# yangcaoai/CoDA_NeurIPS2023

Measured on NVIDIA H100. Metric: training scenes/sec (20k-pt SUN-RGBD synth, 256 queries), higher is better.
Workload: dtype fp32

## Files before the change

### coda_neurips2023_b200/csrc/sa_mlp_kernels.cu

```cuda
#include <cuda_bf16.h>
#include <math.h>
#include <stdint.h>

#include "../../include/coda_sa_mlp.h"
#include "coda_common.cuh"
#include "operand_split.cuh"

namespace {

constexpr int THREADS = 256;
constexpr int MAX_BLOCKS = 132 * 4;

__host__ __device__ inline bool channels_ok(int c) { return c >= 4 && c <= 1024 && c % 4 == 0 && THREADS % (c / 4) == 0; }

__host__ inline unsigned grid_for(long long rows, int c) {
  const long long per_iter = THREADS / (c / 4);
  const long long need = (rows + per_iter - 1) / per_iter;
  return (unsigned)(need < MAX_BLOCKS ? (need > 0 ? need : 1) : MAX_BLOCKS);
}

struct Affine4 {
  float4 mean, invstd, gamma, beta;
};
__device__ __forceinline__ Affine4 load_affine(const float *mean, const float *invstd, const float *gamma,
// ... 146 lines not shown
  warp_partials_sum(nblocks, c, ch, partial, s, q);
  if ((threadIdx.x & 31) != 0) return;
  sums[ch] = s;
  sums[c + ch] = q;
}
__global__ void __launch_bounds__(256)
bn_finalize_sums_kernel(long long rows, int c, int cpad, const double *__restrict__ sums, float eps, float momentum,
                        float *running_mean, float *running_var, const float *__restrict__ gamma,
                        const float *__restrict__ beta, float *__restrict__ mean, float *__restrict__ invstd,
                        float *__restrict__ scale, float *__restrict__ shift) {
  const int ch = blockIdx.x * blockDim.x + threadIdx.x;
  if (ch >= cpad) return;
  if (ch >= c) {
    if (scale) { scale[ch] = 0.f; shift[ch] = 0.f; }
    return;
  }
  const double n = (double)rows, m = sums[ch] / n;
  double var = sums[c + ch] / n - m * m;
  if (var < 0.0) var = 0.0;
  const float is = (float)(1.0 / sqrt(var + (double)eps));
  mean[ch] = (float)m;
  invstd[ch] = is;
  if (running_mean) running_mean[ch] = (1.0f - momentum) * running_mean[ch] + momentum * (float)m;
  if (running_var) running_var[ch] = (1.0f - momentum) * running_var[ch] + momentum * (float)(var * (n / fmax(n - 1.0, 1.0)));
  if (scale) {
    const float sc = gamma[ch] * is;
    scale[ch] = sc;
    shift[ch] = beta[ch] - (float)m * sc;
  }
}

__global__ void bn_bwd_coefs_kernel(int c, int cpad, long long rows, const float *__restrict__ mean,
                                    const float *__restrict__ invstd, const float *__restrict__ gamma,
                                    const float *__restrict__ s1, const float *__restrict__ s2,
                                    float *__restrict__ alpha, float *__restrict__ beta) {
  const int ch = blockIdx.x * blockDim.x + threadIdx.x;
  if (ch >= cpad) return;
  if (ch >= c) { alpha[ch] = 0.f; beta[ch] = 0.f; return; }
  const float inv_n = 1.0f / (float)rows;
  const float sc = gamma[ch] * invstd[ch];
  const float a = -sc * invstd[ch] * (s2[ch] * inv_n);
  alpha[ch] = a;
  beta[ch] = -sc * (s1[ch] * inv_n) - a * mean[ch];
}

__global__ void __launch_bounds__(THREADS)
colsum_partial_kernel(long long rows, int c, const float *__restrict__ x, float *__restrict__ partial) {
  __shared__ float4 red[THREADS];
  const int cq = c >> 2, c4 = threadIdx.x % cq, slot = threadIdx.x / cq, nslots = THREADS / cq;
  float4 acc[1] = {make_float4(0.f, 0.f, 0.f, 0.f)};
  for (long long r = (long long)blockIdx.x * nslots + slot; r < rows; r += (long long)gridDim.x * nslots) {
    const float4 v = __ldg(reinterpret_cast<const float4 *>(x + r * c) + c4);
    acc[0].x += v.x; acc[0].y += v.y; acc[0].z += v.z; acc[0].w += v.w;
  }
  reduce_slots<1>(acc, cq, slot, c4, red);
  if (slot == 0) reinterpret_cast<float4 *>(partial + (size_t)blockIdx.x * c)[c4] = acc[0];
}
__global__ void __launch_bounds__(256)
colsum_finalize_kernel(int nblocks, int c, const float *__restrict__ partial, float *__restrict__ out) {
  const int ch = blockIdx.x * 8 + (threadIdx.x >> 5), lane = threadIdx.x & 31;
  if (ch >= c) return;
  float a = 0.f;
  for (int k = lane; k < nblocks; k += 32) a += partial[(size_t)k * c + ch];
#pragma unroll
  for (int o = 16; o > 0; o >>= 1) a += __shfl_xor_sync(0xffffffffu, a, o);
  if (lane == 0) out[ch] = a;
}

template <int NS>
__global__ void __launch_bounds__(THREADS)
bn_relu_pack_kernel(long long rows, int c, const float *__restrict__ y, const float *__restrict__ mean,
                    const float *__restrict__ invstd, const float *__restrict__ gamma, const float *__restrict__ beta,
                    __nv_bfloat16 *__restrict__ planes) {
  const int cq = c >> 2, c4 = threadIdx.x % cq, slot = threadIdx.x / cq, nslots = THREADS / cq;
  const Affine4 a = load_affine(mean, invstd, gamma, beta, c4);
  const size_t plane_stride = (size_t)rows * c;
  for (long long r = (long long)blockIdx.x * nslots + slot; r < rows; r += (long long)gridDim.x * nslots) {
    const float4 z = bn4(xhat4(__ldg(reinterpret_cast<const float4 *>(y + r * c) + c4), a), a);
    coda::split_store4<NS>(make_float4(fmaxf(z.x, 0.f), fmaxf(z.y, 0.f), fmaxf(z.z, 0.f), fmaxf(z.w, 0.f)),
                           planes + r * c + c4 * 4, plane_stride);
  }
}

__global__ void __launch_bounds__(THREADS)
bn_relu_maxpool_kernel(long long groups, int group, int c, const float *__restrict__ y, const float *__restrict__ mean,
                       const float *__restrict__ invstd, const float *__restrict__ gamma,
                       const float *__restrict__ beta, float *__restrict__ pooled, unsigned char *__restrict__ argmax) {
  __shared__ float4 sval[THREADS];
  __shared__ uchar4 sidx[THREADS];
  const int cq = c >> 2, c4 = threadIdx.x % cq, slot = threadIdx.x / cq, nslots = THREADS / cq;
  const Affine4 a = load_affine(mean, invstd, gamma, beta, c4);
  for (long long g = blockIdx.x; g < groups; g += gridDim.x) {
    float4 best = make_float4(-INFINITY, -INFINITY, -INFINITY, -INFINITY);
    uchar4 bi = make_uchar4(0, 0, 0, 0);
    for (int i = slot; i < group; i += nslots) {
      const float4 zz = bn4(xhat4(__ldg(reinterpret_cast<const float4 *>(y + (g * group + i) * c) + c4), a), a);
      const float4 z = make_float4(fmaxf(zz.x, 0.f), fmaxf(zz.y, 0.f), fmaxf(zz.z, 0.f), fmaxf(zz.w, 0.f));
      if (z.x > best.x) { best.x = z.x; bi.x = (unsigned char)i; }
      if (z.y > best.y) { best.y = z.y; bi.y = (unsigned char)i; }
      if (z.z > best.z) { best.z = z.z; bi.z = (unsigned char)i; }
      if (z.w > best.w) { best.w = z.w; bi.w = (unsigned char)i; }
    }
    __syncthreads();
    sval[threadIdx.x] = best;
    sidx[threadIdx.x] = bi;
    __syncthreads();
    if (slot == 0) {
      for (int s = 1; s < nslots; ++s) {
        const float4 o = sval[s * cq + c4];
        const uchar4 oi = sidx[s * cq + c4];
        if (o.x > best.x || (o.x == best.x && oi.x < bi.x)) { best.x = o.x; bi.x = oi.x; }
        if (o.y > best.y || (o.y == best.y && oi.y < bi.y)) { best.y = o.y; bi.y = oi.y; }
        if (o.z > best.z || (o.z == best.z && oi.z < bi.z)) { best.z = o.z; bi.z = oi.z; }
        if (o.w > best.w || (o.w == best.w && oi.w < bi.w)) { best.w = o.w; bi.w = oi.w; }
      }
      reinterpret_cast<float4 *>(pooled + g * c)[c4] = best;
      reinterpret_cast<uchar4 *>(argmax + g * c)[c4] = bi;
    }
  }
}

__global__ void __launch_bounds__(THREADS)
bn_relu_bwd_reduce_kernel(long long rows, int c, const float *__restrict__ y, const float *__restrict__ dz,
                          const float *__restrict__ mean, const float *__restrict__ invstd,
                          const float *__restrict__ gamma, const float *__restrict__ beta, float *__restrict__ partial) {
  __shared__ float4 red[THREADS];
  const int cq = c >> 2, c4 = threadIdx.x % cq, slot = threadIdx.x / cq, nslots = THREADS / cq;
  const Affine4 a = load_affine(mean, invstd, gamma, beta, c4);
  float4 acc[2] = {make_float4(0.f, 0.f, 0.f, 0.f), make_float4(0.f, 0.f, 0.f, 0.f)};
  for (long long r = (long long)blockIdx.x * nslots + slot; r < rows; r += (long long)gridDim.x * nslots) {
    const float4 xh = xhat4(__ldg(reinterpret_cast<const float4 *>(y + r * c) + c4), a);
    const float4 z = bn4(xh, a);
    float4 d = __ldg(reinterpret_cast<const float4 *>(dz + r * c) + c4);
    d.x = z.x > 0.f ? d.x : 0.f; d.y = z.y > 0.f ? d.y : 0.f; d.z = z.z > 0.f ? d.z : 0.f; d.w = z.w > 0.f ? d.w : 0.f;
    acc[0].x += d.x; acc[0].y += d.y; acc[0].z += d.z; acc[0].w += d.w;
    acc[1].x = fmaf(d.x, xh.x, acc[1].x); acc[1].y = fmaf(d.y, xh.y, acc[1].y);
    acc[1].z = fmaf(d.z, xh.z, acc[1].z); acc[1].w = fmaf(d.w, xh.w, acc[1].w);
  }
  reduce_slots<2>(acc, cq, slot, c4, red);
  if (slot == 0) {
    float4 *p = reinterpret_cast<float4 *>(partial + (size_t)blockIdx.x * 2 * c);
    p[c4] = acc[0];
    p[cq + c4] = acc[1];
  }
}
__global__ void __launch_bounds__(THREADS)
bn_relu_bwd_reduce_pooled_kernel(long long groups, int group, int c, const float *__restrict__ y,
                                 const float *__restrict__ dpooled, const unsigned char *__restrict__ argmax,
                                 const float *__restrict__ mean, const float *__restrict__ invstd,
                                 const float *__restrict__ gamma, const float *__restrict__ beta,
                                 float *__restrict__ partial, float *__restrict__ dprime) {
  __shared__ float4 red[THREADS];
  const int cq = c >> 2, c4 = threadIdx.x % cq, slot = threadIdx.x / cq, nslots = THREADS / cq;
  const Affine4 a = load_affine(mean, invstd, gamma, beta, c4);
  float4 acc[2] = {make_float4(0.f, 0.f, 0.f, 0.f), make_float4(0.f, 0.f, 0.f, 0.f)};
  for (long long g = (long long)blockIdx.x * nslots + slot; g < groups; g += (long long)gridDim.x * nslots) {
    const uchar4 id = __ldg(reinterpret_cast<const uchar4 *>(argmax + g * c) + c4);
    const float *base = y + g * group * c + c4 * 4;
    const float4 v = make_float4(__ldg(base + (size_t)id.x * c), __ldg(base + (size_t)id.y * c + 1),
                                 __ldg(base + (size_t)id.z * c + 2), __ldg(base + (size_t)id.w * c + 3));
    const float4 xh = xhat4(v, a);
    const float4 z = bn4(xh, a);
    float4 d = __ldg(reinterpret_cast<const float4 *>(dpooled + g * c) + c4);
    d.x = z.x > 0.f ? d.x : 0.f; d.y = z.y > 0.f ? d.y : 0.f; d.z = z.z > 0.f ? d.z : 0.f; d.w = z.w > 0.f ? d.w : 0.f;
    if (dprime)
      reinterpret_cast<float4 *>(dprime + g * c)[c4] =
          make_float4(a.gamma.x * a.invstd.x * d.x, a.gamma.y * a.invstd.y * d.y, a.gamma.z * a.invstd.z * d.z,
                      a.gamma.w * a.invstd.w * d.w);
    acc[0].x += d.x; acc[0].y += d.y; acc[0].z += d.z; acc[0].w += d.w;
    acc[1].x = fmaf(d.x, xh.x, acc[1].x); acc[1].y = fmaf(d.y, xh.y, acc[1].y);
    acc[1].z = fmaf(d.z, xh.z, acc[1].z); acc[1].w = fmaf(d.w, xh.w, acc[1].w);
  }
  reduce_slots<2>(acc, cq, slot, c4, red);
  if (slot == 0) {
    float4 *p = reinterpret_cast<float4 *>(partial + (size_t)blockIdx.x * 2 * c);
    p[c4] = acc[0];
    p[cq + c4] = acc[1];
  }
}
__global__ void __launch_bounds__(256)
sums_finalize_kernel(int nblocks, int c, const float *__restrict__ partial, float *__restrict__ s1,
                     float *__restrict__ s2) {
  const int ch = blockIdx.x * 8 + (threadIdx.x >> 5);
  if (ch >= c) return;
  double a, b;
  warp_partials_sum(nblocks, c, ch, partial, a, b);
  if ((threadIdx.x & 31) == 0) {
    s1[ch] = (float)a;
    s2[ch] = (float)b;
  }
}

struct BwdCoef4 {
  float4 k, m1, m2;
};
__device__ __forceinline__ BwdCoef4 load_coef(const Affine4 &a, const float *s1, const float *s2, int c4, float inv_n) {
  const float4 t1 = __ldg(reinterpret_cast<const float4 *>(s1) + c4), t2 = __ldg(reinterpret_cast<const float4 *>(s2) + c4);
  BwdCoef4 q;
  q.k = make_float4(a.gamma.x * a.invstd.x, a.gamma.y * a.invstd.y, a.gamma.z * a.invstd.z, a.gamma.w * a.invstd.w);
  q.m1 = make_float4(t1.x * inv_n, t1.y * inv_n, t1.z * inv_n, t1.w * inv_n);
  q.m2 = make_float4(t2.x * inv_n, t2.y * inv_n, t2.z * inv_n, t2.w * inv_n);
// ... 123 lines not shown
  bn_stats_finalize_affine_kernel<<<(cpad + 7) / 8, 256, 0, s>>>((int)grid, rows, c, cpad, scratch, eps, momentum,
                                                                    running_mean, running_var, gamma, beta, mean,
                                                                    invstd, scale, shift);
  return coda::launch_status();
}

int coda_bn_stats_finalize(int nblocks, long long rows, int c, const float *partial, float eps, float momentum,
                           float *running_mean, float *running_var, const float *gamma, const float *beta,
                           float *mean, float *invstd, float *scale, float *shift, void *stream) {
  if (nblocks <= 0 || rows <= 0 || c <= 0 || !partial || !mean || !invstd) return CODA_EINVAL;
  if ((scale != nullptr) != (shift != nullptr) || (scale && (!gamma || !beta))) return CODA_EINVAL;
  const int cpad = (c + 63) / 64 * 64;
  bn_stats_finalize_affine_kernel<<<(cpad + 7) / 8, 256, 0, (cudaStream_t)stream>>>(
      nblocks, rows, c, cpad, partial, eps, momentum, running_mean, running_var, gamma, beta, mean, invstd, scale, shift);
  return coda::launch_status();
}

int coda_bn_rows_sums(long long rows, int c, const float *y, double *sums, float *scratch, void *stream) {
  if (rows <= 0 || !channels_ok(c) || !y || !sums || !scratch) return CODA_EINVAL;
  cudaStream_t s = (cudaStream_t)stream;
  const unsigned grid = grid_for(rows, c);
  bn_stats_partial_kernel<<<grid, THREADS, 0, s>>>(rows, c, y, scratch);
  bn_sums_f64_kernel<<<(c + 7) / 8, 256, 0, s>>>((int)grid, c, scratch, sums);
  return coda::launch_status();
}

int coda_bn_partials_sums(int nblocks, int c, const float *partial, double *sums, void *stream) {
  if (nblocks <= 0 || c <= 0 || !partial || !sums) return CODA_EINVAL;
  bn_sums_f64_kernel<<<(c + 7) / 8, 256, 0, (cudaStream_t)stream>>>(nblocks, c, partial, sums);
  return coda::launch_status();
}

int coda_bn_stats_finalize_sums(long long rows, int c, const double *sums, float eps, float momentum,
                                float *running_mean, float *running_var, const float *gamma, const float *beta,
                                float *mean, float *invstd, float *scale, float *shift, void *stream) {
  if (rows <= 0 || c <= 0 || !sums || !mean || !invstd) return CODA_EINVAL;
  if ((scale != nullptr) != (shift != nullptr) || (scale && (!gamma || !beta))) return CODA_EINVAL;
  const int cpad = scale ? (c + 63) / 64 * 64 : c;
  bn_finalize_sums_kernel<<<(cpad + 127) / 128, 128, 0, (cudaStream_t)stream>>>(
      rows, c, cpad, sums, eps, momentum, running_mean, running_var, gamma, beta, mean, invstd, scale, shift);
  return coda::launch_status();
}

int coda_bn_bwd_coefs(int c, long long rows, const float *mean, const float *invstd, const float *gamma,
                      const float *s1, const float *s2, float *alpha, float *beta, void *stream) {
  if (c <= 0 || rows <= 0 || !mean || !invstd || !gamma || !s1 || !s2 || !alpha || !beta) return CODA_EINVAL;
  const int cpad = (c + 63) / 64 * 64;
  bn_bwd_coefs_kernel<<<(cpad + 127) / 128, 128, 0, (cudaStream_t)stream>>>(c, cpad, rows, mean, invstd, gamma, s1, s2,
                                                                           alpha, beta);
  return coda::launch_status();
}

int coda_rows_colsum(long long rows, int c, const float *x, float *out, float *scratch, void *stream) {
  if (rows <= 0 || !channels_ok(c) || !x || !out || !scratch) return CODA_EINVAL;
  cudaStream_t s = (cudaStream_t)stream;
  unsigned grid = grid_for(rows, c);
  if (grid > 132) grid = 132;
  colsum_partial_kernel<<<grid, THREADS, 0, s>>>(rows, c, x, scratch);
  colsum_finalize_kernel<<<(c + 7) / 8, 256, 0, s>>>((int)grid, c, scratch, out);
  return coda::launch_status();
}

int coda_bn_relu_pack_rows(long long rows, int c, int nsplit, const float *y, const float *mean,
                           const float *invstd, const float *gamma, const float *beta, void *planes,
                           void *stream) {
  if (rows < 0 || !channels_ok(c) || c % 64 != 0 || nsplit < 1 || nsplit > 3) return CODA_EINVAL;
  if (rows == 0) return CODA_OK;
  if (!y || !mean || !invstd || !gamma || !beta || !planes) return CODA_EINVAL;
  cudaStream_t s = (cudaStream_t)stream;
  const unsigned grid = grid_for(rows, c);
  __nv_bfloat16 *p = (__nv_bfloat16 *)planes;
  if (nsplit == 1) bn_relu_pack_kernel<1><<<grid, THREADS, 0, s>>>(rows, c, y, mean, invstd, gamma, beta, p);
  else if (nsplit == 2) bn_relu_pack_kernel<2><<<grid, THREADS, 0, s>>>(rows, c, y, mean, invstd, gamma, beta, p);
  else bn_relu_pack_kernel<3><<<grid, THREADS, 0, s>>>(rows, c, y, mean, invstd, gamma, beta, p);
  return coda::launch_status();
}

int coda_bn_relu_maxpool_rows(long long groups, int group, int c, const float *y, const float *mean,
                              const float *invstd, const float *gamma, const float *beta, float *pooled,
                              unsigned char *argmax, void *stream) {
  if (groups < 0 || group < 1 || group > 256 || !channels_ok(c)) return CODA_EINVAL;
  if (groups == 0) return CODA_OK;
  if (!y || !mean || !invstd || !gamma || !beta || !pooled || !argmax) return CODA_EINVAL;
  const unsigned grid = (unsigned)(groups < 132 * 8 ? groups : 132 * 8);
  bn_relu_maxpool_kernel<<<grid, THREADS, 0, (cudaStream_t)stream>>>(groups, group, c, y, mean, invstd, gamma, beta,
                                                                    pooled, argmax);
  return coda::launch_status();
}

int coda_bn_relu_bwd_reduce(long long rows, int c, const float *y, const float *dz, const float *mean,
                            const float *invstd, const float *gamma, const float *beta, float *s1, float *s2,
                            float *scratch, void *stream) {
  if (rows <= 0 || !channels_ok(c) || !y || !dz || !mean || !invstd || !gamma || !beta || !s1 || !s2 || !scratch)
    return CODA_EINVAL;
  cudaStream_t s = (cudaStream_t)stream;
  const unsigned grid = grid_for(rows, c);
  bn_relu_bwd_reduce_kernel<<<grid, THREADS, 0, s>>>(rows, c, y, dz, mean, invstd, gamma, beta, scratch);
  sums_finalize_kernel<<<(c + 7) / 8, 256, 0, s>>>((int)grid, c, scratch, s1, s2);
  return coda::launch_status();
}

int coda_bn_relu_bwd_reduce_pooled(long long groups, int group, int c, const float *y, const float *dpooled,
                                   const unsigned char *argmax, const float *mean, const float *invstd,
                                   const float *gamma, const float *beta, float *s1, float *s2, float *scratch,
                                   float *dprime, void *stream) {
  if (groups <= 0 || group < 1 || group > 256 || !channels_ok(c) || !y || !dpooled || !argmax || !mean || !invstd ||
      !gamma || !beta || !s1 || !s2 || !scratch)
    return CODA_EINVAL;
  cudaStream_t s = (cudaStream_t)stream;
  const unsigned grid = grid_for(groups, c);
  bn_relu_bwd_reduce_pooled_kernel<<<grid, THREADS, 0, s>>>(groups, group, c, y, dpooled, argmax, mean, invstd, gamma,
                                                           beta, scratch, dprime);
  sums_finalize_kernel<<<(c + 7) / 8, 256, 0, s>>>((int)grid, c, scratch, s1, s2);
  return coda::launch_status();
}

int coda_bn_relu_bwd_pack(long long rows, int c, int nsplit, const float *y, const float *dz,
                          const float *dpooled, const unsigned char *argmax, int group, const float *mean,
                          const float *invstd, const float *gamma, const float *beta, const float *s1,
                          const float *s2, void *planes, void *stream) {
  if (rows < 0 || !channels_ok(c) || c % 64 != 0 || nsplit < 1 || nsplit > 3) return CODA_EINVAL;
  if (rows == 0) return CODA_OK;
  if (!y || !mean || !invstd || !gamma || !beta || !s1 || !s2 || !planes) return CODA_EINVAL;
  const bool pooled = dz == nullptr;
  if (pooled && (!dpooled || !argmax || group < 1 || group > 256 || rows % group != 0)) return CODA_EINVAL;
  cudaStream_t s = (cudaStream_t)stream;
  const unsigned grid = grid_for(rows, c);
  __nv_bfloat16 *p = (__nv_bfloat16 *)planes;
#define CODA_LAUNCH(NS, P) \
  bn_relu_bwd_pack_kernel<NS, P><<<grid, THREADS, 0, s>>>(rows, c, y, dz, dpooled, argmax, group, mean, invstd, gamma, \
                                                          beta, s1, s2, p)
  if (pooled) {
    if (nsplit == 1) CODA_LAUNCH(1, true); else if (nsplit == 2) CODA_LAUNCH(2, true); else CODA_LAUNCH(3, true);
  } else {
    if (nsplit == 1) CODA_LAUNCH(1, false); else if (nsplit == 2) CODA_LAUNCH(2, false); else CODA_LAUNCH(3, false);
  }
#undef CODA_LAUNCH
  return coda::launch_status();
}

int coda_bn_relu_bwd_small_k(long long rows, int cin, int cout, const float *y, const float *dz, const float *mean,
                             const float *invstd, const float *gamma, const float *beta, const float *s1,
                             const float *s2, const float *x, float *dw, float *scratch, void *stream) {
  if (rows <= 0 || cin < 1 || cin > 8 || !channels_ok(cout)) return CODA_EINVAL;
  if (!y || !dz || !mean || !invstd || !gamma || !beta || !s1 || !s2 || !x || !dw || !scratch) return CODA_EINVAL;
  cudaStream_t s = (cudaStream_t)stream;
  const unsigned grid = grid_for(rows, cout);
#define CODA_CASE(K)                                                                                              \
  case K:                                                                                                         \
    bn_relu_bwd_small_k_kernel<K><<<grid, THREADS, 0, s>>>(rows, cout, y, dz, mean, invstd, gamma, beta, s1, s2, x, \
                                                           scratch);                                             \
    break;
  switch (cin) { CODA_CASE(1) CODA_CASE(2) CODA_CASE(3) CODA_CASE(4) CODA_CASE(5) CODA_CASE(6) CODA_CASE(7) CODA_CASE(8) }
#undef CODA_CASE
  dw_finalize_kernel<<<(cin * cout + 127) / 128, 128, 0, s>>>((int)grid, cin * cout, scratch, dw);
  return coda::launch_status();
}

}
```

### coda_neurips2023_b200/csrc/gemm_sm90.cu

```cuda
#include "../../include/coda_gemm.h"
#include "sm90_primitives.cuh"

using namespace coda;

namespace {

template <int NSPLIT>
__global__ void __launch_bounds__(256)
pack_rows_kernel(long long rows, int k, int kpad, long long src_row_stride, const float *__restrict__ src,
                 float scale, __nv_bfloat16 *__restrict__ planes, long long plane_stride) {
  const long long idx = (long long)blockIdx.x * blockDim.x + threadIdx.x;
  if (idx >= rows * kpad) return;
  const long long r = idx / kpad;
  const int c = (int)(idx - r * kpad);
  const float x = c < k ? __ldg(src + r * src_row_stride + c) * scale : 0.f;
  split_store<NSPLIT>(x, planes + idx, (size_t)plane_stride);
}

template <int NSPLIT>
__global__ void __launch_bounds__(256)
pack_rows_vec4_kernel(long long rows, int k, int kpad, long long src_row_stride, const float *__restrict__ src,
                      float scale, __nv_bfloat16 *__restrict__ planes, long long plane_stride) {
  const int kq = kpad >> 2;
  const long long idx = (long long)blockIdx.x * blockDim.x + threadIdx.x;
// ... 253 lines not shown
      for (int kb = 0; kb < nkb; ++kb, ++it) {
        const int s = it % STAGES;
        mbar_wait(&empty_bar[s], ((it / STAGES) & 1u) ^ 1u);
        if (elect_one_sync()) {
          mbar_arrive_expect_tx(&full_bar[s], (uint32_t)STAGE);
          unsigned char *st = smem + (size_t)s * STAGE;
          tma_load_3d(st, &maps.a[0], &full_bar[s], kb * BK, m0, 0);
          tma_load_3d(st + A_TILE, &maps.b[0], &full_bar[s], kb * BK, n0, 0);
        }
        __syncwarp();
      }
    }
    return;
  }
  setmaxnreg_inc<PP_MMA_REGS>();

  const int wg = warp >> 2, wl = warp & 3;
  const int g = lane >> 2, t = lane & 3;
  float acc[2][BN / 2];
  uint32_t it = (uint32_t)(wg * nkb);
  for (int w = blockIdx.x + wg * gridDim.x; w < ntiles; w += 2 * gridDim.x, it += 2 * nkb) {
    int m0, n0;
    decode(w, m0, n0);
    const bool other_next = w + (int)gridDim.x < ntiles;
    if (wg == 1 || w != (int)blockIdx.x) bar_sync(1 + wg, 256);
    for (int kb = 0; kb < nkb; ++kb) {
      const uint32_t i = it + kb;
      const int s = i % STAGES;
      mbar_wait(&full_bar[s], (i / STAGES) & 1u);
      unsigned char *st = smem + (size_t)s * STAGE;
      acc_fence(acc[0]);
      acc_fence(acc[1]);
      wgmma_fence();
      const uint64_t ad = gmma_desc_k_sw128(st), bd = gmma_desc_k_sw128(st + A_TILE);
#pragma unroll
      for (int kk = 0; kk < BK / 16; ++kk) {
        const uint64_t b = gmma_desc_advance(bd, kk * 32);
        Wgmma<BN, true>::template ss<0, 0>(acc[0], gmma_desc_advance(ad, kk * 32), b, (kb | kk) != 0);
        Wgmma<BN, true>::template ss<0, 0>(acc[1], gmma_desc_advance(ad, 8192 + kk * 32), b, (kb | kk) != 0);
      }
      wgmma_commit();
      if (kb == nkb - 1 && other_next) bar_arrive(1 + (wg ^ 1), 256);
      wgmma_wait<1>();
      acc_fence(acc[0]);
      acc_fence(acc[1]);
      if (kb > 0 && (threadIdx.x & 127) == 0) mbar_arrive(&empty_bar[(i - 1) % STAGES]);
    }

    float2 bv[BN / 8];
    if (EPI != PP_NONE) {
#pragma unroll
      for (int cc = 0; cc < BN / 8; ++cc) bv[cc] = __ldg(reinterpret_cast<const float2 *>(bias + n0 + cc * 8 + 2 * t));
    }
    wgmma_wait<0>();
    acc_fence(acc[0]);
    acc_fence(acc[1]);
    if ((threadIdx.x & 127) == 0) mbar_arrive(&empty_bar[(it + nkb - 1) % STAGES]);

#pragma unroll
    for (int h = 0; h < 2; ++h) {
#pragma unroll
      for (int r = 0; r < 2; ++r) {
        const int row = m0 + h * 64 + wl * 16 + g + 8 * r;
        if (row >= m) continue;
        __half *crow = c + (size_t)row * ldc + n0 + 2 * t;
        const __half *rrow = EPI == PP_BIAS_RES ? residual + (size_t)row * ldr + n0 + 2 * t : nullptr;
#pragma unroll
        for (int cc = 0; cc < BN / 8; ++cc) {
          float v0 = acc[h][cc * 4 + r * 2], v1 = acc[h][cc * 4 + r * 2 + 1];
          if (EPI != PP_NONE) { v0 += bv[cc].x; v1 += bv[cc].y; }
          if (EPI == PP_BIAS_GELU) { v0 = apply_act(v0, 2); v1 = apply_act(v1, 2); }
          if (EPI == PP_BIAS_RES) {
            const __half2 rv = *reinterpret_cast<const __half2 *>(rrow + cc * 8);
            v0 += __low2float(rv);
            v1 += __high2float(rv);
          }
          *reinterpret_cast<__half2 *>(crow + cc * 8) = __floats2half2_rn(v0, v1);
        }
      }
    }
  }
}

template <int NSPLIT, int BN, int STAGES, bool FP16, bool MN = false>
int launch_gemm(const GemmMaps &maps, int batch, int m, int n, int kpad, int b_batched, const float *bias, int relu,
                void *c_out, long long ldc, long long c_batch_stride, cudaStream_t s, int out_half = 0,
                const void *residual = nullptr, long long ldr = 0) {
  float *c = reinterpret_cast<float *>(c_out);
  const int sms = sm_count();
  const long long tiles = (long long)((m + BM - 1) / BM) * ((n + BN - 1) / BN) * batch;
  const int nkb_total = kpad / BK;
  int ksplit = 1;
  if (!relu && !out_half && tiles < sms && nkb_total >= 32) {
    ksplit = (int)((2 * sms + tiles - 1) / tiles);
    if (ksplit > nkb_total / 8) ksplit = nkb_total / 8;
    if (ksplit < 1) ksplit = 1;
    const int per = (nkb_total + ksplit - 1) / ksplit;
    ksplit = (nkb_total + per - 1) / per;
  }
  if (residual && (!FP16 || !out_half || batch != 1 || (ldr & 7) != 0 || ((uintptr_t)residual & 15) != 0))
    return CODA_EINVAL;
  float *partial = nullptr;
  if (ksplit > 1) {
    const int st = split_scratch((size_t)tiles * ksplit * BM * BN, s, &partial);
    if (st != CODA_OK) return st;
  }
  constexpr size_t smem = (size_t)STAGES * NSPLIT * (BM * BK * 2 + BN * BK * 2) + 1024;
  static_assert(smem <= 227 * 1024, "smem budget");
  constexpr auto kern = gemm_nt_kernel<NSPLIT, BN, STAGES, FP16, MN>;
  if (const int st = raise_smem_limit<kern>((int)smem)) return st;
  const long long nwork = tiles * ksplit;
  const unsigned grid = (unsigned)(nwork < sms ? nwork : sms);
  kern<<<grid, GEMM_THREADS, smem, s>>>(maps, m, n, kpad, b_batched, ksplit, batch, bias, relu, out_half, c_out, ldc,
                                        c_batch_stride, residual, ldr, partial);
  if (ksplit > 1) {
    const long long total = (long long)batch * m * n;
    const long long blocks = (total + 255) / 256;
    splitk_reduce_kernel<<<(unsigned)(blocks < 8 * sms ? blocks : 8 * sms), 256, 0, s>>>(partial, ksplit, m, n, batch, BM,
                                                                                          BN, bias, c, ldc, c_batch_stride);
  }
  return launch_status();
}

template <int BN, int STAGES, int EPI>
int launch_gemm_f16_pp(const GemmMaps &maps, int m, int n, int kpad, const float *bias, const void *residual,
                       long long ldr, void *c, long long ldc, cudaStream_t s) {
  constexpr size_t smem = (size_t)STAGES * (BM * BK * 2 + BN * BK * 2) + 1024;
  static_assert(smem <= 227 * 1024, "smem budget");
  constexpr auto kern = gemm_f16_pp_kernel<BN, STAGES, EPI>;
  if (const int st = raise_smem_limit<kern>((int)smem)) return st;
  const int sms = sm_count();
  const int tiles = (m + BM - 1) / BM * (n / BN);
  kern<<<(unsigned)(tiles < sms ? tiles : sms), PP_THREADS, smem, s>>>(
      maps, m, n, kpad / BK, bias, reinterpret_cast<const __half *>(residual), ldr, reinterpret_cast<__half *>(c), ldc);
  return launch_status();
}

}

extern "C" {

int coda_pack_split_bf16_strided(long long rows, int k, int kpad, long long src_row_stride,
                                 long long src_k_stride, const float *src, float scale, int nsplit, void *planes,
                                 long long plane_stride, void *stream) {
  if (rows < 0 || k < 0 || kpad < k || kpad % 64 != 0 || nsplit < 1 || nsplit > 3) return CODA_EINVAL;
  if (rows == 0 || kpad == 0) return CODA_OK;
  if (!src || !planes) return CODA_EINVAL;
  cudaStream_t s = (cudaStream_t)stream;
  __nv_bfloat16 *out = (__nv_bfloat16 *)planes;
  if ((src_k_stride == 1 || k <= 1) && k % 4 == 0 && src_row_stride % 4 == 0 && ((uintptr_t)src & 15) == 0 &&
      plane_stride % 4 == 0 && ((uintptr_t)out & 7) == 0) {
    const long long total = rows * (kpad / 4);
    const unsigned grid = (unsigned)((total + 255) / 256);
    if (nsplit == 1) pack_rows_vec4_kernel<1><<<grid, 256, 0, s>>>(rows, k, kpad, src_row_stride, src, scale, out, plane_stride);
    else if (nsplit == 2) pack_rows_vec4_kernel<2><<<grid, 256, 0, s>>>(rows, k, kpad, src_row_stride, src, scale, out, plane_stride);
    else pack_rows_vec4_kernel<3><<<grid, 256, 0, s>>>(rows, k, kpad, src_row_stride, src, scale, out, plane_stride);
  } else if (src_k_stride == 1 || k <= 1) {
    const long long total = rows * kpad;
    const unsigned grid = (unsigned)((total + 255) / 256);
    if (nsplit == 1) pack_rows_kernel<1><<<grid, 256, 0, s>>>(rows, k, kpad, src_row_stride, src, scale, out, plane_stride);
    else if (nsplit == 2) pack_rows_kernel<2><<<grid, 256, 0, s>>>(rows, k, kpad, src_row_stride, src, scale, out, plane_stride);
    else pack_rows_kernel<3><<<grid, 256, 0, s>>>(rows, k, kpad, src_row_stride, src, scale, out, plane_stride);
  } else if (src_row_stride == 1) {
    const dim3 grid((unsigned)((rows + 31) / 32), (kpad + 31) / 32);
    if (grid.y > 65535) return CODA_ETOOLARGE;
    if (nsplit == 1) pack_transposed_kernel<1><<<grid, 256, 0, s>>>(rows, k, kpad, src_k_stride, src, scale, out, plane_stride);
    else if (nsplit == 2) pack_transposed_kernel<2><<<grid, 256, 0, s>>>(rows, k, kpad, src_k_stride, src, scale, out, plane_stride);
    else pack_transposed_kernel<3><<<grid, 256, 0, s>>>(rows, k, kpad, src_k_stride, src, scale, out, plane_stride);
  } else {
    return CODA_EINVAL;
  }
  return launch_status();
}

int coda_pack_split_bf16(long long rows, int k, int kpad, long long src_row_stride, long long src_k_stride,
                         const float *src, float scale, int nsplit, void *planes, void *stream) {
  return coda_pack_split_bf16_strided(rows, k, kpad, src_row_stride, src_k_stride, src, scale, nsplit, planes,
                                      rows * kpad, stream);
}

int coda_gemm_nt(int nsplit, int is_fp16, int batch, int m, int n, int kpad, const void *a,
                 long long a_plane_stride, long long a_batch_stride, const void *b, long long b_plane_stride,
                 long long b_batch_stride, const float *bias, int relu, float *c, long long ldc,
                 long long c_batch_stride, void *stream) {
  return coda_gemm_nt_ex(nsplit, is_fp16, batch, m, n, kpad, a, a_plane_stride, a_batch_stride, b, b_plane_stride,
                         b_batch_stride, bias, relu, 0, c, ldc, c_batch_stride, stream);
}

int coda_gemm_nt_ex(int nsplit, int is_fp16, int batch, int m, int n, int kpad, const void *a,
                    long long a_plane_stride, long long a_batch_stride, const void *b, long long b_plane_stride,
                    long long b_batch_stride, const float *bias, int relu, int out_half, void *c, long long ldc,
                    long long c_batch_stride, void *stream) {
  return coda_gemm_nt_res(nsplit, is_fp16, batch, m, n, kpad, a, a_plane_stride, a_batch_stride, b, b_plane_stride,
                          b_batch_stride, bias, relu, out_half, nullptr, 0, c, ldc, c_batch_stride, stream);
}

int coda_gemm_nt_res(int nsplit, int is_fp16, int batch, int m, int n, int kpad, const void *a,
                     long long a_plane_stride, long long a_batch_stride, const void *b, long long b_plane_stride,
                     long long b_batch_stride, const float *bias, int relu, int out_half, const void *residual,
                     long long ldr, void *c, long long ldc, long long c_batch_stride, void *stream) {
  if (nsplit < 1 || nsplit > 3 || batch < 0 || m < 0 || n < 0 || kpad < 0 || kpad % 64 != 0) return CODA_EINVAL;
  if (is_fp16 && nsplit != 1) return CODA_EINVAL;
  if (batch == 0 || m == 0 || n == 0) return CODA_OK;
  if (!a || !b || !c || kpad == 0 || batch > 65535) return CODA_EINVAL;
  constexpr int PP_BN = 128;
  const int pp_epi = !bias ? (relu == 0 && !residual ? PP_NONE : -1)
                     : relu == 0 ? (residual ? PP_BIAS_RES : PP_BIAS)
                     : (relu == 2 && !residual) ? PP_BIAS_GELU : -1;
  const long long pp_tiles = (long long)((m + BM - 1) / BM) * (n / PP_BN);
  const bool pp = is_fp16 && out_half && batch == 1 && pp_epi >= 0 && n % PP_BN == 0 &&
                  pp_tiles >= 2LL * sm_count() && pp_tiles <= INT_MAX && ldc % 8 == 0 &&
                  ((uintptr_t)c & 15) == 0 && ((uintptr_t)bias & 7) == 0 &&
                  (!residual || (ldr % 8 == 0 && ((uintptr_t)residual & 15) == 0));
  const int bn = pp ? PP_BN
                 : n <= 64 ? 64
                 : (is_fp16 && n % 256 == 0 && n >= 1536) ? 256
                 : (is_fp16 && n % 192 == 0 && n >= 384)  ? 192
                                                          : 128;
  GemmMaps maps;
  const char *ap = (const char *)a, *bp = (const char *)b;
  for (int p = 0; p < nsplit; ++p) {
    int st = make_tmap_k_major_16b(&maps.a[p], ap + (size_t)p * a_plane_stride * 2, is_fp16, kpad, m, batch, kpad,
                                   a_batch_stride, BM);
    if (st != CODA_OK) return st;
    st = make_tmap_k_major_16b(&maps.b[p], bp + (size_t)p * b_plane_stride * 2, is_fp16, kpad, n,
                               b_batch_stride ? batch : 1, kpad, b_batch_stride, bn);
    if (st != CODA_OK) return st;
  }
  cudaStream_t s = (cudaStream_t)stream;
  const int bb = b_batch_stride ? 1 : 0;
#define CODA_GEMM(NS, BN_, ST, F16) \
  return launch_gemm<NS, BN_, ST, F16>(maps, batch, m, n, kpad, bb, bias, relu, c, ldc, c_batch_stride, s, out_half, \
                                       residual, ldr)
  if (pp) {
#define CODA_GEMM_PP(EPI) \
  return launch_gemm_f16_pp<PP_BN, 6, EPI>(maps, m, n, kpad, bias, residual, ldr, c, ldc, s)
    if (pp_epi == PP_NONE) CODA_GEMM_PP(PP_NONE);
    if (pp_epi == PP_BIAS) CODA_GEMM_PP(PP_BIAS);
    if (pp_epi == PP_BIAS_GELU) CODA_GEMM_PP(PP_BIAS_GELU);
    CODA_GEMM_PP(PP_BIAS_RES);
#undef CODA_GEMM_PP
  }
  if (is_fp16) {
    if (bn == 64) CODA_GEMM(1, 64, 6, true);
    if (bn == 256) CODA_GEMM(1, 256, 4, true);
    if (bn == 192) CODA_GEMM(1, 192, 5, true);
    CODA_GEMM(1, 128, 6, true);
  }
  if (nsplit == 1) {
    if (bn == 64) CODA_GEMM(1, 64, 6, false);
    CODA_GEMM(1, 128, 6, false);
  }
  if (nsplit == 2) {
    if (bn == 64) CODA_GEMM(2, 64, 4, false);
    CODA_GEMM(2, 128, 3, false);
  }
  if (bn == 64) CODA_GEMM(3, 64, 2, false);
  CODA_GEMM(3, 128, 2, false);
#undef CODA_GEMM
}


int coda_gemm_tn(int nsplit, int mc, int m, int n, const void *a, long long a_plane_stride, int lda,
                 const void *b, long long b_plane_stride, int ldb, float *c, long long ldc, void *stream) {
  if (nsplit < 1 || nsplit > 3 || mc < 0 || m < 0 || n < 0 || lda % 64 != 0 || ldb % 64 != 0) return CODA_EINVAL;
  if (m == 0 || n == 0) return CODA_OK;
  if (!a || !b || !c || mc == 0 || lda < m || ldb < n) return CODA_EINVAL;
  const int bn = n <= 64 ? 64 : 128;
  GemmMaps maps;
  const char *ap = (const char *)a, *bp = (const char *)b;
  for (int p = 0; p < nsplit; ++p) {
    int st = make_tmap_k_major_16b(&maps.a[p], ap + (size_t)p * a_plane_stride * 2, 0, lda, mc, 1, lda, 0, 64);
    if (st != CODA_OK) return st;
    st = make_tmap_k_major_16b(&maps.b[p], bp + (size_t)p * b_plane_stride * 2, 0, ldb, mc, 1, ldb, 0, 64);
    if (st != CODA_OK) return st;
  }
  cudaStream_t s = (cudaStream_t)stream;
  const int kpad = (mc + 63) / 64 * 64;
#define CODA_GEMM_TN(NS, BN_, ST) \
  return launch_gemm<NS, BN_, ST, false, true>(maps, 1, m, n, kpad, 0, nullptr, 0, c, ldc, 0, s)
  if (nsplit == 1) { if (bn == 64) CODA_GEMM_TN(1, 64, 6); CODA_GEMM_TN(1, 128, 6); }
  if (nsplit == 2) { if (bn == 64) CODA_GEMM_TN(2, 64, 4); CODA_GEMM_TN(2, 128, 3); }
  if (bn == 64) CODA_GEMM_TN(3, 64, 2);
  CODA_GEMM_TN(3, 128, 2);
#undef CODA_GEMM_TN
}

}
```

Before: 199.6.

## Give each thread slot a whole group in maxpool and batch row loads

The fused BN+ReLU+maxpool kernel now assigns one group per thread slot instead of spreading a group's rows across slots. This removes the shared-memory cross-slot reduction and its two block barriers per group. Rows are loaded 16 at a time into registers so more memory requests are in flight, and the grid is sized by groups per block. The costs are higher register pressure and less parallelism when there are few groups. Tie-breaking now follows the sequential scan order only.

```diff
diff --git a/coda_neurips2023_b200/csrc/sa_mlp_kernels.cu b/coda_neurips2023_b200/csrc/sa_mlp_kernels.cu
--- a/coda_neurips2023_b200/csrc/sa_mlp_kernels.cu
+++ b/coda_neurips2023_b200/csrc/sa_mlp_kernels.cu
@@ -252,41 +252,36 @@
   }
 }
 
+constexpr int MAXPOOL_ROWS_IN_FLIGHT = 16;
 __global__ void __launch_bounds__(THREADS)
 bn_relu_maxpool_kernel(long long groups, int group, int c, const float *__restrict__ y, const float *__restrict__ mean,
                        const float *__restrict__ invstd, const float *__restrict__ gamma,
                        const float *__restrict__ beta, float *__restrict__ pooled, unsigned char *__restrict__ argmax) {
-  __shared__ float4 sval[THREADS];
-  __shared__ uchar4 sidx[THREADS];
   const int cq = c >> 2, c4 = threadIdx.x % cq, slot = threadIdx.x / cq, nslots = THREADS / cq;
   const Affine4 a = load_affine(mean, invstd, gamma, beta, c4);
-  for (long long g = blockIdx.x; g < groups; g += gridDim.x) {
+  for (long long g = (long long)blockIdx.x * nslots + slot; g < groups; g += (long long)gridDim.x * nslots) {
+    const float4 *rows = reinterpret_cast<const float4 *>(y + g * group * c) + c4;
     float4 best = make_float4(-INFINITY, -INFINITY, -INFINITY, -INFINITY);
     uchar4 bi = make_uchar4(0, 0, 0, 0);
-    for (int i = slot; i < group; i += nslots) {
-      const float4 zz = bn4(xhat4(__ldg(reinterpret_cast<const float4 *>(y + (g * group + i) * c) + c4), a), a);
-      const float4 z = make_float4(fmaxf(zz.x, 0.f), fmaxf(zz.y, 0.f), fmaxf(zz.z, 0.f), fmaxf(zz.w, 0.f));
-      if (z.x > best.x) { best.x = z.x; bi.x = (unsigned char)i; }
-      if (z.y > best.y) { best.y = z.y; bi.y = (unsigned char)i; }
-      if (z.z > best.z) { best.z = z.z; bi.z = (unsigned char)i; }
-      if (z.w > best.w) { best.w = z.w; bi.w = (unsigned char)i; }
+    for (int i0 = 0; i0 < group; i0 += MAXPOOL_ROWS_IN_FLIGHT) {
+      float4 v[MAXPOOL_ROWS_IN_FLIGHT];
+#pragma unroll
+      for (int u = 0; u < MAXPOOL_ROWS_IN_FLIGHT; ++u)
+        if (i0 + u < group) v[u] = __ldg(rows + (size_t)(i0 + u) * cq);
+#pragma unroll
+      for (int u = 0; u < MAXPOOL_ROWS_IN_FLIGHT; ++u) {
+        if (i0 + u >= group) break;
+        const float4 zz = bn4(xhat4(v[u], a), a);
+        const float4 z = make_float4(fmaxf(zz.x, 0.f), fmaxf(zz.y, 0.f), fmaxf(zz.z, 0.f), fmaxf(zz.w, 0.f));
+        const unsigned char i = (unsigned char)(i0 + u);
+        if (z.x > best.x) { best.x = z.x; bi.x = i; }
+        if (z.y > best.y) { best.y = z.y; bi.y = i; }
+        if (z.z > best.z) { best.z = z.z; bi.z = i; }
+        if (z.w > best.w) { best.w = z.w; bi.w = i; }
+      }
     }
-    __syncthreads();
-    sval[threadIdx.x] = best;
-    sidx[threadIdx.x] = bi;
-    __syncthreads();
-    if (slot == 0) {
-      for (int s = 1; s < nslots; ++s) {
-        const float4 o = sval[s * cq + c4];
-        const uchar4 oi = sidx[s * cq + c4];
-        if (o.x > best.x || (o.x == best.x && oi.x < bi.x)) { best.x = o.x; bi.x = oi.x; }
-        if (o.y > best.y || (o.y == best.y && oi.y < bi.y)) { best.y = o.y; bi.y = oi.y; }
-        if (o.z > best.z || (o.z == best.z && oi.z < bi.z)) { best.z = o.z; bi.z = oi.z; }
-        if (o.w > best.w || (o.w == best.w && oi.w < bi.w)) { best.w = o.w; bi.w = oi.w; }
-      }
-      reinterpret_cast<float4 *>(pooled + g * c)[c4] = best;
-      reinterpret_cast<uchar4 *>(argmax + g * c)[c4] = bi;
-    }
+    reinterpret_cast<float4 *>(pooled + g * c)[c4] = best;
+    reinterpret_cast<uchar4 *>(argmax + g * c)[c4] = bi;
   }
 }
 
@@ -576,7 +571,8 @@
   if (groups < 0 || group < 1 || group > 256 || !channels_ok(c)) return CODA_EINVAL;
   if (groups == 0) return CODA_OK;
   if (!y || !mean || !invstd || !gamma || !beta || !pooled || !argmax) return CODA_EINVAL;
-  const unsigned grid = (unsigned)(groups < 132 * 8 ? groups : 132 * 8);
+  const long long blocks = (groups + THREADS / (c / 4) - 1) / (THREADS / (c / 4));
+  const unsigned grid = (unsigned)(blocks < 132 * 8 ? blocks : 132 * 8);
   bn_relu_maxpool_kernel<<<grid, THREADS, 0, (cudaStream_t)stream>>>(groups, group, c, y, mean, invstd, gamma, beta,
                                                                     pooled, argmax);
   return coda::launch_status();
```

After: 198.9 (median of 6 runs). No clear change (-0.3%).

## Add cooperative persistent fp16 GEMM with wide N tiles and smem-staged epilogue

Applied to the files above, without the earlier changes.

Adds a warp-specialized persistent fp16 GEMM in which both consumer warpgroups share one wide B tile (192 or 256 columns) and split the 128-row M tile. Output is staged through shared memory so global stores are coalesced 16-byte writes. The dispatcher picks this kernel for eligible non-residual fp16 half-output GEMMs, choosing the width with the smaller per-SM column load, and falls back to the ping-pong kernel otherwise. The goal is more reuse per loaded tile and better wave balance, at the cost of losing ping-pong overlap between epilogue and MMA and using more registers per thread.

```diff
diff --git a/coda_neurips2023_b200/csrc/gemm_sm90.cu b/coda_neurips2023_b200/csrc/gemm_sm90.cu
--- a/coda_neurips2023_b200/csrc/gemm_sm90.cu
+++ b/coda_neurips2023_b200/csrc/gemm_sm90.cu
@@ -359,6 +359,115 @@
   }
 }
 
+constexpr int COOP_EP_LD = 72;
+constexpr size_t COOP_EP_SMEM = 8 * 16 * COOP_EP_LD * 2;
+template <int BN, int STAGES, int EPI>
+__global__ void __launch_bounds__(PP_THREADS, 1)
+gemm_f16_coop_kernel(const __grid_constant__ GemmMaps maps, int m, int n, int nkb, const float *__restrict__ bias,
+                     const __half *__restrict__, long long, __half *__restrict__ c, long long ldc) {
+  static_assert(EPI != PP_BIAS_RES, "no residual epilogue");
+  constexpr int A_TILE = BM * BK * 2;
+  constexpr int STAGE = A_TILE + BN * BK * 2;
+  extern __shared__ __align__(1024) unsigned char smem_raw[];
+  unsigned char *smem = smem_align1024(smem_raw);
+  __shared__ __align__(8) uint64_t full_bar[STAGES];
+  __shared__ __align__(8) uint64_t empty_bar[STAGES];
+
+  const int warp = threadIdx.x >> 5, lane = threadIdx.x & 31;
+  const int tiles_m = (m + BM - 1) / BM, tiles_n = n / BN;
+  const int ntiles = tiles_m * tiles_n;
+  const bool n_fast = tiles_n <= tiles_m;
+  auto decode = [&](int w, int &m0, int &n0) {
+    const int tm = n_fast ? w / tiles_n : w % tiles_m, tn = n_fast ? w % tiles_n : w / tiles_m;
+    m0 = tm * BM; n0 = tn * BN;
+  };
+
+  if (threadIdx.x == 0) {
+    for (int s = 0; s < STAGES; ++s) { mbar_init(&full_bar[s], 1); mbar_init(&empty_bar[s], 2); }
+    mbar_fence_init_cluster();
+  }
+  __syncthreads();
+
+  if (warp >= 8) {
+    setmaxnreg_dec<PP_PRODUCER_REGS>();
+    if (warp != 8) return;
+    if (lane == 0) { prefetch_tmap(&maps.a[0]); prefetch_tmap(&maps.b[0]); }
+    uint32_t it = 0;
+    for (int w = blockIdx.x; w < ntiles; w += gridDim.x) {
+      int m0, n0;
+      decode(w, m0, n0);
+      for (int kb = 0; kb < nkb; ++kb, ++it) {
+        const int s = it % STAGES;
+        mbar_wait(&empty_bar[s], ((it / STAGES) & 1u) ^ 1u);
+        if (elect_one_sync()) {
+          mbar_arrive_expect_tx(&full_bar[s], (uint32_t)STAGE);
+          unsigned char *st = smem + (size_t)s * STAGE;
+          tma_load_3d(st, &maps.a[0], &full_bar[s], kb * BK, m0, 0);
+          tma_load_3d(st + A_TILE, &maps.b[0], &full_bar[s], kb * BK, n0, 0);
+        }
+        __syncwarp();
+      }
+    }
+    return;
+  }
+  setmaxnreg_inc<PP_MMA_REGS>();
+
+  const int wg = warp >> 2, wl = warp & 3;
+  const int g = lane >> 2, t = lane & 3;
+  __half *ep = reinterpret_cast<__half *>(smem + STAGES * STAGE) + warp * 16 * COOP_EP_LD;
+  float acc[BN / 2];
+  uint32_t it = 0;
+  for (int w = blockIdx.x; w < ntiles; w += gridDim.x) {
+    int m0, n0;
+    decode(w, m0, n0);
+    for (int kb = 0; kb < nkb; ++kb, ++it) {
+      const int s = it % STAGES;
+      mbar_wait(&full_bar[s], (it / STAGES) & 1u);
+      unsigned char *st = smem + (size_t)s * STAGE;
+      acc_fence(acc);
+      wgmma_fence();
+      const uint64_t ad = gmma_desc_k_sw128(st + wg * 8192), bd = gmma_desc_k_sw128(st + A_TILE);
+#pragma unroll
+      for (int kk = 0; kk < BK / 16; ++kk)
+        Wgmma<BN, true>::template ss<0, 0>(acc, gmma_desc_advance(ad, kk * 32), gmma_desc_advance(bd, kk * 32),
+                                           (kb | kk) != 0);
+      wgmma_commit();
+      wgmma_wait<1>();
+      acc_fence(acc);
+      if (kb > 0 && (threadIdx.x & 127) == 0) mbar_arrive(&empty_bar[(it - 1) % STAGES]);
+    }
+    wgmma_wait<0>();
+    acc_fence(acc);
+    if ((threadIdx.x & 127) == 0) mbar_arrive(&empty_bar[(it - 1) % STAGES]);
+
+#pragma unroll
+    for (int q = 0; q < BN / 64; ++q) {
+#pragma unroll
+      for (int c8 = 0; c8 < 8; ++c8) {
+        const int cc = q * 8 + c8;
+        float2 bv = make_float2(0.f, 0.f);
+        if (EPI != PP_NONE) bv = __ldg(reinterpret_cast<const float2 *>(bias + n0 + cc * 8 + 2 * t));
+#pragma unroll
+        for (int r = 0; r < 2; ++r) {
+          float v0 = acc[cc * 4 + r * 2], v1 = acc[cc * 4 + r * 2 + 1];
+          if (EPI != PP_NONE) { v0 += bv.x; v1 += bv.y; }
+          if (EPI == PP_BIAS_GELU) { v0 = apply_act(v0, 2); v1 = apply_act(v1, 2); }
+          *reinterpret_cast<__half2 *>(ep + (g + 8 * r) * COOP_EP_LD + c8 * 8 + 2 * t) = __floats2half2_rn(v0, v1);
+        }
+      }
+      __syncwarp();
+#pragma unroll
+      for (int j = 0; j < 4; ++j) {
+        const int rl = j * 4 + (lane >> 3), ch = lane & 7;
+        const uint4 v = *reinterpret_cast<const uint4 *>(ep + rl * COOP_EP_LD + ch * 8);
+        const int grow = m0 + wg * 64 + wl * 16 + rl;
+        if (grow < m) *reinterpret_cast<uint4 *>(c + (size_t)grow * ldc + n0 + q * 64 + ch * 8) = v;
+      }
+      __syncwarp();
+    }
+  }
+}
+
 template <int NSPLIT, int BN, int STAGES, bool FP16, bool MN = false>
 int launch_gemm(const GemmMaps &maps, int batch, int m, int n, int kpad, int b_batched, const float *bias, int relu,
                 void *c_out, long long ldc, long long c_batch_stride, cudaStream_t s, int out_half = 0,
@@ -399,12 +508,18 @@
   return launch_status();
 }
 
-template <int BN, int STAGES, int EPI>
-int launch_gemm_f16_pp(const GemmMaps &maps, int m, int n, int kpad, const float *bias, const void *residual,
-                       long long ldr, void *c, long long ldc, cudaStream_t s) {
-  constexpr size_t smem = (size_t)STAGES * (BM * BK * 2 + BN * BK * 2) + 1024;
+template <bool COOP, int BN, int STAGES, int EPI>
+constexpr auto f16_kernel() {
+  if constexpr (COOP) return gemm_f16_coop_kernel<BN, STAGES, EPI>;
+  else return gemm_f16_pp_kernel<BN, STAGES, EPI>;
+}
+
+template <bool COOP, int BN, int STAGES, int EPI>
+int launch_gemm_f16(const GemmMaps &maps, int m, int n, int kpad, const float *bias, const void *residual,
+                    long long ldr, void *c, long long ldc, cudaStream_t s) {
+  constexpr size_t smem = (size_t)STAGES * (BM * BK * 2 + BN * BK * 2) + (COOP ? COOP_EP_SMEM : 0) + 1024;
   static_assert(smem <= 227 * 1024, "smem budget");
-  constexpr auto kern = gemm_f16_pp_kernel<BN, STAGES, EPI>;
+  constexpr auto kern = f16_kernel<COOP, BN, STAGES, EPI>();
   if (const int st = raise_smem_limit<kern>((int)smem)) return st;
   const int sms = sm_count();
   const int tiles = (m + BM - 1) / BM * (n / BN);
@@ -484,12 +599,23 @@
   const int pp_epi = !bias ? (relu == 0 && !residual ? PP_NONE : -1)
                      : relu == 0 ? (residual ? PP_BIAS_RES : PP_BIAS)
                      : (relu == 2 && !residual) ? PP_BIAS_GELU : -1;
-  const long long pp_tiles = (long long)((m + BM - 1) / BM) * (n / PP_BN);
-  const bool pp = is_fp16 && out_half && batch == 1 && pp_epi >= 0 && n % PP_BN == 0 &&
-                  pp_tiles >= 2LL * sm_count() && pp_tiles <= INT_MAX && ldc % 8 == 0 &&
-                  ((uintptr_t)c & 15) == 0 && ((uintptr_t)bias & 7) == 0 &&
-                  (!residual || (ldr % 8 == 0 && ((uintptr_t)residual & 15) == 0));
-  const int bn = pp ? PP_BN
+  const bool f16_ok = is_fp16 && out_half && batch == 1 && pp_epi >= 0 && ldc % 8 == 0 &&
+                      ((uintptr_t)c & 15) == 0 && ((uintptr_t)bias & 7) == 0 &&
+                      (!residual || (ldr % 8 == 0 && ((uintptr_t)residual & 15) == 0));
+  const int tiles_m = (m + BM - 1) / BM;
+  auto coop_cols = [&](int w) -> long long {
+    const long long tiles = (long long)tiles_m * (n / w);
+    return n % w || n / w < 4 || tiles > INT_MAX ? LLONG_MAX : (tiles + sm_count() - 1) / sm_count() * w;
+  };
+  const long long cols256 = coop_cols(256), cols192 = coop_cols(192);
+  const int coop_bn = !f16_ok || residual ? 0
+                      : cols192 != LLONG_MAX && cols192 <= cols256 ? 192
+                      : cols256 != LLONG_MAX ? 256 : 0;
+  const bool coop = coop_bn != 0;
+  const long long pp_tiles = (long long)tiles_m * (n / PP_BN);
+  const bool pp = !coop && f16_ok && n % PP_BN == 0 && pp_tiles >= 2LL * sm_count() && pp_tiles <= INT_MAX;
+  const int bn = coop ? coop_bn
+                 : pp ? PP_BN
                  : n <= 64 ? 64
                  : (is_fp16 && n % 256 == 0 && n >= 1536) ? 256
                  : (is_fp16 && n % 192 == 0 && n >= 384)  ? 192
@@ -509,15 +635,25 @@
 #define CODA_GEMM(NS, BN_, ST, F16) \
   return launch_gemm<NS, BN_, ST, F16>(maps, batch, m, n, kpad, bb, bias, relu, c, ldc, c_batch_stride, s, out_half, \
                                        residual, ldr)
+#define CODA_GEMM_F16(COOP, BN_, ST, EPI) \
+  return launch_gemm_f16<COOP, BN_, ST, EPI>(maps, m, n, kpad, bias, residual, ldr, c, ldc, s)
+  if (coop) {
+    if (bn == 256) {
+      if (pp_epi == PP_NONE) CODA_GEMM_F16(true, 256, 4, PP_NONE);
+      if (pp_epi == PP_BIAS) CODA_GEMM_F16(true, 256, 4, PP_BIAS);
+      CODA_GEMM_F16(true, 256, 4, PP_BIAS_GELU);
+    }
+    if (pp_epi == PP_NONE) CODA_GEMM_F16(true, 192, 5, PP_NONE);
+    if (pp_epi == PP_BIAS) CODA_GEMM_F16(true, 192, 5, PP_BIAS);
+    CODA_GEMM_F16(true, 192, 5, PP_BIAS_GELU);
+  }
   if (pp) {
-#define CODA_GEMM_PP(EPI) \
-  return launch_gemm_f16_pp<PP_BN, 6, EPI>(maps, m, n, kpad, bias, residual, ldr, c, ldc, s)
-    if (pp_epi == PP_NONE) CODA_GEMM_PP(PP_NONE);
-    if (pp_epi == PP_BIAS) CODA_GEMM_PP(PP_BIAS);
-    if (pp_epi == PP_BIAS_GELU) CODA_GEMM_PP(PP_BIAS_GELU);
-    CODA_GEMM_PP(PP_BIAS_RES);
-#undef CODA_GEMM_PP
-  }
+    if (pp_epi == PP_NONE) CODA_GEMM_F16(false, PP_BN, 6, PP_NONE);
+    if (pp_epi == PP_BIAS) CODA_GEMM_F16(false, PP_BN, 6, PP_BIAS);
+    if (pp_epi == PP_BIAS_GELU) CODA_GEMM_F16(false, PP_BN, 6, PP_BIAS_GELU);
+    CODA_GEMM_F16(false, PP_BN, 6, PP_BIAS_RES);
+  }
+#undef CODA_GEMM_F16
   if (is_fp16) {
     if (bn == 64) CODA_GEMM(1, 64, 6, true);
     if (bn == 256) CODA_GEMM(1, 256, 4, true);
```

New measurement: 199.1 before, 200.0 after (median of 6 runs). About the same (+0.5%).
